# lz4/lz4-java

Measured on NVIDIA H100. Metric: lz4_fast_compress_plus_decompress_64KiB_blocks, higher is better.
Workload: dtype u8

## Files before the change

### lz4-java_b200/csrc/lz4_compress_wide.cuh

```cuda
#pragma once
#include "common.cuh"
#include "lz4_emit.cuh"
#include <type_traits>

namespace b200 {

#ifdef B200_HOST_SIM
__device__ __forceinline__ void wide_bar_arrive(int id) { simt::bar_arrive(id, 64); }
__device__ __forceinline__ void wide_bar_wait(int id) { simt::bar_sync(id, 64); }
__device__ __forceinline__ uint32_t ldg_u32(const uint32_t* p) { return *p; }
__device__ __forceinline__ void ldg_pair(const uint32_t* base, uint32_t idx, uint32_t& lo, uint32_t& hi) { lo = base[idx]; hi = base[idx + 1]; }
__device__ __forceinline__ uint2 ldg_u64(const uint2* p) { return *p; }
#else
#define B200_WBAR_CASE(OP, N) case N: asm volatile(OP " " #N ", 64;" ::: "memory"); break;
__device__ __forceinline__ void wide_bar_arrive(int id)
{
    switch (id) { B200_WBAR_CASE("bar.arrive", 1) B200_WBAR_CASE("bar.arrive", 2) B200_WBAR_CASE("bar.arrive", 3)
                  B200_WBAR_CASE("bar.arrive", 4) B200_WBAR_CASE("bar.arrive", 5) default: asm volatile("bar.arrive 6, 64;" ::: "memory"); }
}
__device__ __forceinline__ void wide_bar_wait(int id)
{
    switch (id) { B200_WBAR_CASE("bar.sync", 1) B200_WBAR_CASE("bar.sync", 2) B200_WBAR_CASE("bar.sync", 3)
                  B200_WBAR_CASE("bar.sync", 4) B200_WBAR_CASE("bar.sync", 5) default: asm volatile("bar.sync 6, 64;" ::: "memory"); }
}
__device__ __forceinline__ uint32_t ldg_u32(const uint32_t* p) { return __ldg(p); }
__device__ __forceinline__ uint2 ldg_u64(const uint2* p) { return __ldg(p); }
__device__ __forceinline__ void ldg_pair(const uint32_t* base, uint32_t idx, uint32_t& lo, uint32_t& hi)
{
    uint64_t a;
    asm("mad.wide.u32 %0, %1, 4, %2;" : "=l"(a) : "r"(idx), "l"(base));
    asm("ld.global.nc.u32 %0, [%1];" : "=r"(lo) : "l"(a));
    asm("ld.global.nc.u32 %0, [%1+4];" : "=r"(hi) : "l"(a));
}
#endif

template <int S, int NB, int NW>
struct WideLayout {
    static constexpr int CH = 128 * S;
    static constexpr int MW = CH / 32;
    static constexpr int BUF_BYTES = CH * 3 + MW * 4;
    static constexpr int REC_BYTES = 32 * 8 + 16;
    static constexpr size_t smem(int hash_log) { return (size_t(2) << hash_log) + size_t(NB) * BUF_BYTES + REC_BYTES; }
};

template <int HASH_LOG, int S, int NB, int NW, int MINB>
__global__ void __launch_bounds__(32 * NW, MINB)
lz4_compress_wide_kernel(const uint8_t* __restrict__ src_base, const uint64_t* __restrict__ src_off,
                         const int32_t* __restrict__ src_len,
                         uint8_t* __restrict__ dst_base, const uint64_t* __restrict__ dst_off,
                         const int32_t* __restrict__ dst_cap, int32_t* __restrict__ result, uint32_t nblocks)
{
    using LY = WideLayout<S, NB, NW>;
    constexpr int CH = LY::CH, MW = LY::MW;
    constexpr int TABLE_BYTES = 2 << HASH_LOG;
    constexpr int BAR_FULL = 1, BAR_FREE = 1 + NB, BAR_REC_FULL = 1 + 2 * NB, BAR_REC_FREE = 2 + 2 * NB;
    constexpr int REC_LAST = 0x100;
    static_assert(NW == 2 || NW == 3, "two or three warps");
    static_assert(2 * NB + (NW == 3 ? 2 : 0) <= 6, "named barrier ids 1..6");
    B200_DYN_SMEM(smem_raw, 128);
    uint16_t* table = reinterpret_cast<uint16_t*>(smem_raw);
    uint8_t* bufs = smem_raw + TABLE_BYTES;
    auto dist_of = [&](int buf) { return reinterpret_cast<uint16_t*>(bufs + buf * LY::BUF_BYTES); };
    auto flen_of = [&](int buf) { return bufs + buf * LY::BUF_BYTES + CH * 2; };
    auto hmask_of = [&](int buf) { return reinterpret_cast<uint32_t*>(bufs + buf * LY::BUF_BYTES + CH * 3); };
    uint2* s_rec = reinterpret_cast<uint2*>(bufs + NB * LY::BUF_BYTES);
    int* s_hdr = reinterpret_cast<int*>(bufs + NB * LY::BUF_BYTES + 256);

    const uint32_t b = blockIdx.x;
    if (b >= nblocks) return;
    const int lane = lane_id();
    const int role = threadIdx.x >> 5;
    const uint8_t* __restrict__ src = src_base + src_off[b];
    uint8_t* __restrict__ dst = dst_base + dst_off[b];
    const int n = src_len[b];
    const int cap = dst_cap[b];

    if (n < 0 || n >= 65536 + 11 || cap < 0) { if (threadIdx.x == 0) result[b] = 0; return; }
    if (n == 0) { if (threadIdx.x == 0) { if (cap >= 1) dst[0] = 0; result[b] = cap >= 1 ? 1 : 0; } return; }

    const uint32_t ph = uint32_t(reinterpret_cast<uintptr_t>(src)) & 3u;
    const uint32_t* __restrict__ wsrc = reinterpret_cast<const uint32_t*>(reinterpret_cast<uintptr_t>(src) - ph);
    const uint32_t ph8 = uint32_t(reinterpret_cast<uintptr_t>(src)) & 7u;
    const uint2* __restrict__ qsrc = reinterpret_cast<const uint2*>(reinterpret_cast<uintptr_t>(src) - ph8);
    const int mflimit = n - 12, matchlimit = n - 5;
    const int nchunks = mflimit >= 0 ? (mflimit + int(ph)) / CH + 1 : 0;
    auto ld4 = [&](int pos) -> uint32_t {
        const uint32_t a = uint32_t(pos) + ph;
        uint32_t lo, hi;
        ldg_pair(wsrc, a >> 2, lo, hi);
        return __funnelshift_r(lo, hi, a << 3);
    };

    if (role == 0) {
        for (int i = lane; i < TABLE_BYTES / 16; i += 32) reinterpret_cast<uint4*>(table)[i] = make_uint4(0, 0, 0, 0);
        __syncwarp();
        auto lookup = [&](int c, auto edge_tag) {
            constexpr bool EDGE = decltype(edge_tag)::value;
            const int buf = c % NB;
            const int cp0 = CH * c - int(ph);
            uint32_t w0[S], w1[S], w2[S]; int cand[S][4];
            #pragma unroll
            for (int s = 0; s < S; s++) {
                const int p0 = cp0 + 128 * s + 4 * lane;
                const uint32_t* wp = wsrc + (uint32_t(CH / 4) * uint32_t(c) + 32u * uint32_t(s) + uint32_t(lane));
                w0[s] = w1[s] = w2[s] = 0;
                if (!EDGE || (p0 + 3 >= 0 && p0 <= mflimit)) { w0[s] = ldg_u32(wp); w1[s] = ldg_u32(wp + 1); w2[s] = ldg_u32(wp + 2); }
            }
            #pragma unroll
            for (int s = 0; s < S; s++) {
                const int p0 = cp0 + 128 * s + 4 * lane;
                uint32_t h[4];
                #pragma unroll
                for (int j = 0; j < 4; j++) {
                    const uint32_t sq = j ? __funnelshift_r(w0[s], w1[s], 8 * j) : w0[s];
                    h[j] = (sq * 2654435761u) >> (32 - HASH_LOG);
                    cand[s][j] = table[h[j]];
                }
                __syncwarp();
                #pragma unroll
                for (int j = 0; j < 4; j++) {
                    const int p = p0 + j;
                    if (!EDGE || (p >= 0 && p <= mflimit)) table[h[j]] = uint16_t(p);
                }
                __syncwarp();
            }
            if (c >= NB) wide_bar_wait(BAR_FREE + buf);
            uint16_t* ds = dist_of(buf);
            uint8_t* fls = flen_of(buf);
            uint32_t* hm = hmask_of(buf);
            uint32_t fl[S][4], gh[S];
            #pragma unroll
            for (int s = 0; s < S; s++) {
                const int p0 = cp0 + 128 * s + 4 * lane;
                uint32_t dd[4], nib = 0;
                #pragma unroll
                for (int j = 0; j < 4; j++) {
                    const int p = p0 + j;
                    const uint32_t sq = j ? __funnelshift_r(w0[s], w1[s], 8 * j) : w0[s];
                    const uint32_t sn = j ? __funnelshift_r(w1[s], w2[s], 8 * j) : w1[s];
                    const bool plaus = !EDGE || (p >= 0 && p <= mflimit && cand[s][j] < p);
                    const uint32_t a = uint32_t(plaus ? cand[s][j] : 0) + ph8;
                    const uint2* w = qsrc + (a >> 3);
                    const uint2 q0 = ldg_u64(w), q1 = ldg_u64(w + 1);
                    const bool up = (a & 4u) != 0;
                    const uint32_t c0 = up ? q0.y : q0.x, c1 = up ? q1.x : q0.y, c2 = up ? q1.y : q1.x;
                    const uint32_t x = __funnelshift_r(c0, c1, a << 3) ^ sq;
                    const uint32_t y = __funnelshift_r(c1, c2, a << 3) ^ sn;
                    dd[j] = EDGE ? (uint32_t(p - cand[s][j]) & 0xFFFFu) : uint32_t(p - cand[s][j]);
                    fl[s][j] = 4u + min((uint32_t(__ffs(int(y))) - 1u) >> 3, 4u);
                    if (EDGE) fl[s][j] = uint32_t(min(int(fl[s][j]), max(matchlimit - p, 4)));
                    nib |= uint32_t(plaus && x == 0) << j;
                }
                reinterpret_cast<uint2*>(ds + 128 * s)[lane] = make_uint2(dd[0] | (dd[1] << 16), dd[2] | (dd[3] << 16));
                uint32_t g = nib << (4u * (uint32_t(lane) & 7u));
                g |= __shfl_xor_sync(B200_FULL, g, 1); g |= __shfl_xor_sync(B200_FULL, g, 2); g |= __shfl_xor_sync(B200_FULL, g, 4);
                if ((lane & 7) == 0) hm[4 * s + (lane >> 3)] = g;
                gh[s] = g;
            }
            #pragma unroll
            for (int s = 0; s < S; s++) {
                uint32_t nx = __shfl_down_sync(B200_FULL, gh[s], 8);
                const uint32_t nxs = (s + 1 < S) ? __shfl_sync(B200_FULL, gh[(s + 1) % S], 0) : 0u;
                if (lane >= 24) nx = nxs;
                const uint32_t win = __funnelshift_rc(gh[s], nx, 4u * (uint32_t(lane) & 7u) + 4u);
                uint32_t out = 0;
                #pragma unroll
                for (int j = 0; j < 4; j++) {
                    const uint32_t f = fl[s][j];
                    const uint32_t mm = win >> (uint32_t(j) + f - 4u);
                    const uint32_t z = uint32_t(__ffs(int(mm))) - 1u;
                    const uint32_t code = min(f * 64u - 256u + (z < 32u ? f + z : 0u), 0xFFu);
                    out |= code << (8 * j);
                }
                reinterpret_cast<uint32_t*>(fls + 128 * s)[lane] = out;
            }
            wide_bar_arrive(BAR_FULL + buf);
        };
        for (int c = 0; c < nchunks; c++) {
            const int cp0 = CH * c - int(ph);
            if (lane < S) {
                const int pfq = cp0 + 2 * CH + lane * 128;
                if (pfq < n) B200_PREFETCH_L2(src + pfq);
            }
            if (c > 0 && cp0 + CH - 1 < mflimit) lookup(c, std::false_type{});
            else lookup(c, std::true_type{});
        }
        return;
    }

    int ip = 0;
    int op = 0; bool fail = false;
    int k = 0;
    int r_pend = 0, r_ms = 0, r_len = 4, r_dist = 1;

    auto extend = [&](int a, int dist, int maxlen) -> int {
        int total = 0;
        for (;;) {
            const int i = total + 4 * lane;
            uint32_t x = 1;
            if (i < maxlen) x = ld4(a + i) ^ ld4(a + i - dist);
            const unsigned neq = __ballot_sync(B200_FULL, x != 0);
            if (neq) {
                const int fl = __ffs(neq) - 1;
                const uint32_t xf = __shfl_sync(B200_FULL, x, fl);
                return min(total + 4 * fl + ((__ffs(xf) - 1) >> 3), maxlen);
            }
            total += 128;
        }
    };

    auto layout = [&](int cnt) {
        const bool on = lane < cnt;
        int start = r_ms, len = r_len;
        if (on && r_ms - r_dist >= 4 && r_ms > r_pend) {
            const uint32_t x = ld4(r_ms - 4) ^ ld4(r_ms - r_dist - 4);
            const int back = x ? (__clz(x) >> 3) : 4;
            const int bk = min(back, r_ms - r_pend);
            start -= bk; len += bk;
        }
        const int lit = on ? start - r_pend : 0, mcode = len - 4;
        const int lhdr = lit >= 15 ? (lit - 15) / 255 + 1 : 0;
        const int mhdr = (on && mcode >= 15) ? (mcode - 15) / 255 + 1 : 0;
        const int size = on ? 1 + lhdr + lit + 2 + mhdr : 0;
        int incl = size;
        #pragma unroll
        for (int d = 1; d < 32; d <<= 1) { const int y = __shfl_up_sync(B200_FULL, incl, d); if (lane >= d) incl += y; }
        const int total = __shfl_sync(B200_FULL, incl, 31);
        if (fail) return;
        if (uint32_t(op) + uint32_t(total) > uint32_t(cap)) { fail = true; return; }
        const int o = op + incl - size;
        if (on) {
            uint8_t* d = dst + o;
            d[0] = uint8_t((min(lit, 15) << 4) | min(mcode, 15));
            d += 1;
            if (lit >= 15) { int v = lit - 15; for (; v >= 255; v -= 255) *d++ = 255; *d++ = uint8_t(v); }
            d += lit;
            d[0] = uint8_t(r_dist); d[1] = uint8_t(r_dist >> 8);
            d += 2;
            if (mcode >= 15) { int v = mcode - 15; for (; v >= 255; v -= 255) *d++ = 255; *d++ = uint8_t(v); }
        }
        uint8_t* lo = dst + o + 1 + lhdr;
        const int sn = min(lit, 32);
        const int mx = __reduce_max_sync(B200_FULL, sn);
        for (int t = 0; t < mx; t += 4) {
            if (t < sn) {
                const uint32_t v = ld4(r_pend + t);
                lo[t] = uint8_t(v);
                if (t + 1 < sn) lo[t + 1] = uint8_t(v >> 8);
                if (t + 2 < sn) lo[t + 2] = uint8_t(v >> 16);
                if (t + 3 < sn) lo[t + 3] = uint8_t(v >> 24);
            }
        }
        for (unsigned lm = __ballot_sync(B200_FULL, lit > 32); lm; lm &= lm - 1) {
            const int j = __ffs(lm) - 1;
            const int ka = __shfl_sync(B200_FULL, r_pend, j);
            const int kl = __shfl_sync(B200_FULL, lit, j);
            const int ko = __shfl_sync(B200_FULL, o + 1 + lhdr, j);
            warp_copy(dst + ko + 32, src + ka + 32, kl - 32, lane);
        }
        op += total;
    };

    auto finish = [&](int fin) {
        int ret = 0;
        if (!fail) {
            const int lit = n - fin;
            const int lhdr = lit >= 15 ? (lit - 15) / 255 + 1 : 0;
            if (uint32_t(op) + 1u + uint32_t(lhdr) + uint32_t(lit) <= uint32_t(cap)) {
                if (lane == 0) dst[op] = uint8_t(min(lit, 15) << 4);
                op += 1;
                if (lhdr) { write_len_ext(dst + op, lit - 15, lhdr, lane); op += lhdr; }
                warp_copy(dst + op, src + fin, lit, lane);
                ret = op + lit;
            }
        }
        if (lane == 0) result[b] = ret;
    };

    int prev_end = 0;
    auto layout_batch = [&](int cnt) {
        uint2 r = make_uint2(0, 4);
        if (lane < cnt) r = s_rec[lane];
        if (NW == 3) wide_bar_arrive(BAR_REC_FREE);
        r_ms = int(r.x & 0xFFFFu); r_dist = int(r.x >> 16); r_len = int(r.y);
        const int end = r_ms + r_len;
        r_pend = __shfl_up_sync(B200_FULL, end, 1);
        if (lane == 0) r_pend = prev_end;
        if (cnt > 0) prev_end = __shfl_sync(B200_FULL, end, cnt - 1);
        layout(cnt);
    };

    if (NW == 3 && role == 2) {
        for (;;) {
            wide_bar_wait(BAR_REC_FULL);
            const int hdr = s_hdr[0], fin = s_hdr[1];
            layout_batch(hdr & 0xFF);
            if (hdr & REC_LAST) { finish(fin); break; }
        }
        return;
    }

    auto flush = [&](bool last) {
        if (NW == 2) { __syncwarp(); layout_batch(k); k = 0; __syncwarp(); return; }
        if (lane == 0) { s_hdr[0] = k | (last ? REC_LAST : 0); s_hdr[1] = ip; }
        wide_bar_arrive(BAR_REC_FULL);
        wide_bar_wait(BAR_REC_FREE);
        k = 0;
    };
    for (int c = 0; c < nchunks; c++) {
        const int buf = c % NB;
        const int cp0 = CH * c - int(ph);
        wide_bar_wait(BAR_FULL + buf);
        const uint16_t* ds = dist_of(buf);
        const uint8_t* fls = flen_of(buf);
        const uint32_t* hm = hmask_of(buf);
        auto search = [&](uint32_t r) -> uint32_t {
            if (r >= uint32_t(CH)) return CH;
            uint32_t w = r >> 5;
            uint32_t m = hm[w] & (0xFFFFFFFFu << (r & 31u));
            while (m == 0 && ++w < uint32_t(MW)) m = hm[w];
            return m ? 32u * w + uint32_t(__ffs(int(m))) - 1u : uint32_t(CH);
        };
        uint32_t q = search(uint32_t(max(ip - cp0, 0)));
        uint32_t code = 0, dist = 0;
        if (q < uint32_t(CH)) { code = fls[q]; dist = ds[q]; }
        while (q < uint32_t(CH)) {
            const uint32_t ms = uint32_t(cp0) + q;
            uint32_t fl = 4u + (code >> 6);
            const uint32_t delta = code & 63u;
            uint32_t nq = q + delta;
            if (delta - 1u >= 62u) {
                if (delta) fl = 8u + uint32_t(extend(int(ms) + 8, int(dist), matchlimit - (int(ms) + 8)));
                nq = search(q + fl);
            }
            const uint32_t ncode = fls[nq], ndist = ds[nq];
            if (lane == 0) s_rec[k] = make_uint2(ms | (dist << 16), fl);
            ip = int(ms + fl);
            q = nq; code = ncode; dist = ndist;
            if (++k == 32) flush(false);
        }
        if (c + NB < nchunks) wide_bar_arrive(BAR_FREE + buf);
    }
    flush(true);
    if (NW == 2) finish(ip);
}

}
```

### lz4-java_b200/csrc/lz4_compress.cu

```cuda
#include "common.cuh"
#include "kernels.h"
#include "lz4_emit.cuh"
#include "lz4_compress_wide.cuh"
#include <type_traits>
#include <algorithm>

#ifndef B200_WIDE_WARPS
#define B200_WIDE_WARPS 3
#endif

namespace b200 {

template <int HASH_LOG, bool U16>
__global__ void __launch_bounds__(32)
lz4_compress_long_kernel(const uint8_t* __restrict__ src_base, const uint64_t* __restrict__ src_off,
                          const int32_t* __restrict__ src_len,
                          uint8_t* __restrict__ dst_base, const uint64_t* __restrict__ dst_off,
                          const int32_t* __restrict__ dst_cap, int32_t* __restrict__ result, uint32_t nblocks)
{
    using Entry = typename std::conditional<U16, uint16_t, uint32_t>::type;
    constexpr int TABLE_BYTES = int(sizeof(Entry) << HASH_LOG);
    B200_DYN_SMEM(smem_raw, 128);
    Entry* table = reinterpret_cast<Entry*>(smem_raw);
    uint16_t* s_dist = reinterpret_cast<uint16_t*>(smem_raw + TABLE_BYTES);

    const uint32_t b = blockIdx.x;
    if (b >= nblocks) return;
    const int lane = lane_id();
    const uint8_t* __restrict__ src = src_base + src_off[b];
    uint8_t* __restrict__ dst = dst_base + dst_off[b];
    const int n = src_len[b];
    const int cap = dst_cap[b];
    int ret = 0;

    if (n < 0 || n > 0x7E000000 || cap < 0) goto done;
    if (U16 && n >= 65536 + 11) goto done;
    if (n == 0) { if (cap >= 1) { if (lane == 0) dst[0] = 0; ret = 1; } goto done; }
    {
        for (int i = lane; i < TABLE_BYTES / 16; i += 32) reinterpret_cast<uint4*>(table)[i] = make_uint4(0, 0, 0, 0);
        __syncwarp();
        const uint32_t ph = uint32_t(reinterpret_cast<uintptr_t>(src)) & 3u;
        const uint32_t* __restrict__ wsrc = reinterpret_cast<const uint32_t*>(reinterpret_cast<uintptr_t>(src) - ph);
        auto ld4 = [&](int pos) -> uint32_t {
            const uint32_t a = uint32_t(pos) + ph;
            const uint32_t* w = wsrc + (a >> 2);
            return __funnelshift_r(w[0], w[1], (a & 3u) * 8u);
        };
        const int mflimit = n - 12, matchlimit = n - 5;
        int op = 0, anchor = 0, ip = 0;
        int nrec = 0, r_o = 0, r_lit = 0, r_ml = 0, r_dist = 0;

        auto flush = [&]() {
            if (lane < nrec) {
                const int mcode = r_ml - 4;
                uint8_t* d = dst + r_o;
                d[0] = uint8_t((min(r_lit, 15) << 4) | min(mcode, 15));
                d += 1;
                if (r_lit >= 15) { int v = r_lit - 15; for (; v >= 255; v -= 255) *d++ = 255; *d++ = uint8_t(v); }
                d += r_lit;
                d[0] = uint8_t(r_dist); d[1] = uint8_t(r_dist >> 8);
                d += 2;
                if (mcode >= 15) { int v = mcode - 15; for (; v >= 255; v -= 255) *d++ = 255; *d++ = uint8_t(v); }
            }
            nrec = 0;
        };

        const int nchunks = (mflimit + int(ph)) / 128 + 1;
        for (int c = 0; c < nchunks; c++) {
            const int cp0 = 128 * c - int(ph);
            if (lane < 2) {
                const int pfq = cp0 + 512 + lane * 128;
                if (pfq < n) B200_PREFETCH_L2(src + pfq);
            }
            const int p0 = cp0 + 4 * lane;
            uint32_t w0 = 0, w1 = 0;
            if (p0 + 3 >= 0 && p0 <= mflimit) { w0 = wsrc[32 * c + lane]; w1 = wsrc[32 * c + lane + 1]; }
            uint32_t seq[4], h[4]; int cand[4]; bool plaus[4];
            seq[0] = w0; seq[1] = __funnelshift_r(w0, w1, 8); seq[2] = __funnelshift_r(w0, w1, 16); seq[3] = __funnelshift_r(w0, w1, 24);
            #pragma unroll
            for (int j = 0; j < 4; j++) { h[j] = (seq[j] * 2654435761u) >> (32 - HASH_LOG); cand[j] = table[h[j]]; }
            __syncwarp();
            #pragma unroll
            for (int j = 0; j < 4; j++) {
                const int p = p0 + j;
                const bool valid = p >= 0 && p <= mflimit;
                if (valid) table[h[j]] = Entry(p);
                plaus[j] = valid && cand[j] < p && (U16 || p - cand[j] <= 65535);
            }
            uint32_t cseq[4];
            #pragma unroll
            for (int j = 0; j < 4; j++) cseq[j] = plaus[j] ? ld4(cand[j]) : ~seq[j];
            uint32_t nib = 0; uint32_t d01, d23;
            {
                uint32_t dd[4];
                #pragma unroll
                for (int j = 0; j < 4; j++) {
                    const bool hit = cseq[j] == seq[j];
                    dd[j] = hit ? uint32_t(p0 + j - cand[j]) : 0u;
                    nib |= uint32_t(hit) << j;
                }
                d01 = dd[0] | (dd[1] << 16); d23 = dd[2] | (dd[3] << 16);
            }
            reinterpret_cast<uint2*>(s_dist)[lane] = make_uint2(d01, d23);
            uint32_t gw = nib << (4 * (lane & 7));
            gw |= __shfl_xor_sync(B200_FULL, gw, 1); gw |= __shfl_xor_sync(B200_FULL, gw, 2); gw |= __shfl_xor_sync(B200_FULL, gw, 4);
            const uint32_t hw0 = __shfl_sync(B200_FULL, gw, 0), hw1 = __shfl_sync(B200_FULL, gw, 8),
                           hw2 = __shfl_sync(B200_FULL, gw, 16), hw3 = __shfl_sync(B200_FULL, gw, 24);
            const unsigned long long hlo = (unsigned long long)hw0 | ((unsigned long long)hw1 << 32);
            const unsigned long long hhi = (unsigned long long)hw2 | ((unsigned long long)hw3 << 32);
            __syncwarp();
            for (;;) {
                int r = ip - cp0;
                if (r < 0) r = 0;
                if (r >= 128) break;
                int q;
                {
                    const unsigned long long lo = r < 64 ? (hlo >> r) : 0ull;
                    if (lo) q = r + __ffsll((long long)lo) - 1;
                    else {
                        const int r2 = max(r - 64, 0);
                        const unsigned long long hi = hhi >> r2;
                        if (hi == 0) break;
                        q = 64 + r2 + __ffsll((long long)hi) - 1;
                    }
                }
                int ms = cp0 + q;
                const int dist = s_dist[q];
                int mc = ms - dist, ml;
                {
                    const int d = lane - 8;
                    const int backroom = min(ms - anchor, mc);
                    const bool ok = d < 0 ? (-d <= backroom) : (ms + d < matchlimit);
                    const bool eq = ok && src[ms + d] == src[mc + d];
                    const unsigned e = __ballot_sync(B200_FULL, eq);
                    const int back = __clz((~e) & 0xFFu) - 24;
                    const int fwd = __ffs((~(e >> 8)) | (1u << 24)) - 1;
                    ml = fwd;
                    if (fwd == 24) ml += match_extend(InGlobal{src}, ms + 24, mc + 24, matchlimit - (ms + 24), lane);
                    ms -= back; ml += back;
                }
                const int lit = ms - anchor, mcode = ml - 4;
                const int lhdr = lit >= 15 ? (lit - 15) / 255 + 1 : 0;
                const int mhdr = mcode >= 15 ? (mcode - 15) / 255 + 1 : 0;
                const int size = 1 + lhdr + lit + 2 + mhdr;
                if (uint32_t(op) + uint32_t(size) > uint32_t(cap)) goto done;
                warp_copy(dst + op + 1 + lhdr, src + anchor, lit, lane);
                if (lane == nrec) { r_o = op; r_lit = lit; r_ml = ml; r_dist = dist; }
                nrec++;
                if (nrec == 32) flush();
                op += size;
                ip = anchor = ms + ml;
            }
        }
        flush();
        {
            const int lit = n - anchor;
            const int lhdr = lit >= 15 ? (lit - 15) / 255 + 1 : 0;
            if ((long long)op + 1 + lhdr + lit > cap) goto done;
            if (lane == 0) dst[op] = uint8_t(min(lit, 15) << 4);
            op += 1;
            if (lhdr) { write_len_ext(dst + op, lit - 15, lhdr, lane); op += lhdr; }
            warp_copy(dst + op, src + anchor, lit, lane);
            op += lit;
        }
        ret = op;
    }
done:
    if (lane == 0) result[b] = ret;
}

#ifndef B200_HOST_SIM
template <int HASH_LOG, bool U16>
static cudaError_t launch_long(const BatchArgs& a, cudaStream_t st)
{
    const size_t smem = ((U16 ? 2u : 4u) << HASH_LOG) + 128 * sizeof(uint16_t);
    auto k = lz4_compress_long_kernel<HASH_LOG, U16>;
    cudaError_t e = cudaFuncSetAttribute(k, cudaFuncAttributeMaxDynamicSharedMemorySize, (int)smem);
    if (e != cudaSuccess) return e;
    cudaFuncSetAttribute(k, cudaFuncAttributePreferredSharedMemoryCarveout, cudaSharedmemCarveoutMaxShared);
    k<<<(unsigned)a.n, 32, smem, st>>>(a.src_base, a.src_off, a.src_len, a.dst_base, a.dst_off, a.dst_cap,
                                       a.result, (uint32_t)a.n);
    return cudaGetLastError();
}
#endif


#ifndef B200_HOST_SIM
template <int HASH_LOG, int NB, int NW>
static cudaError_t launch_wide(const BatchArgs& a, cudaStream_t st)
{
    constexpr int S = 2;
    using LY = WideLayout<S, NB, NW>;
    const size_t smem = LY::smem(HASH_LOG);
    constexpr int FIT = 233472 / (int(LY::smem(HASH_LOG)) + 1024);
    constexpr int MINB = FIT < 16 ? FIT : 16;
    auto k = lz4_compress_wide_kernel<HASH_LOG, S, NB, NW, MINB>;
    cudaError_t e = cudaFuncSetAttribute(k, cudaFuncAttributeMaxDynamicSharedMemorySize, (int)smem);
    if (e != cudaSuccess) return e;
    cudaFuncSetAttribute(k, cudaFuncAttributePreferredSharedMemoryCarveout, cudaSharedmemCarveoutMaxShared);
    k<<<(unsigned)a.n, 32 * NW, smem, st>>>(a.src_base, a.src_off, a.src_len, a.dst_base, a.dst_off, a.dst_cap, a.result, (uint32_t)a.n);
    return cudaGetLastError();
}


cudaError_t launch_compress_fast(const BatchArgs& a, int max_src_len, cudaStream_t st)
{
    if (a.n == 0) return cudaSuccess;
    if (max_src_len > 0 && max_src_len <= 65536) return launch_wide<13, 2, B200_WIDE_WARPS>(a, st);
    return launch_long<12, false>(a, st);
}
#endif

}
```

Before: 62.75.

## Replace per-position match bitmap handoff with compacted match-entry lists

The lookup warp now compacts the verified match candidates of each chunk into a packed list. Each entry holds position, distance, length and a skip count. Previously it wrote dense per-position distance, code and hit-mask arrays. The parse warp walks this list and uses a ballot scan to find the next entry, replacing the bitmap word search. This cuts shared-memory traffic and the skipping logic in the serial parse loop, at the cost of ballots and prefix counts in the producer plus an extra split handoff when a chunk has too many hits. Optional clock instrumentation macros are added but compiled out by default.

Result: no change. 63.18, median of 6 (+0.7%).

```diff
diff --git a/lz4-java_b200/csrc/lz4_compress_wide.cuh b/lz4-java_b200/csrc/lz4_compress_wide.cuh
--- a/lz4-java_b200/csrc/lz4_compress_wide.cuh
+++ b/lz4-java_b200/csrc/lz4_compress_wide.cuh
@@ -34,11 +34,23 @@
 }
 #endif
 
+enum { WCLK_L_TOTAL, WCLK_L_FREE, WCLK_P_TOTAL, WCLK_P_FULL, WCLK_P_EXTEND, WCLK_P_SEARCH, WCLK_P_REC_FREE, WCLK_E_REC_FULL, WCLK_N };
+#ifdef B200_WIDE_CLOCKS
+__device__ unsigned long long* b200_wide_clocks;
+#define WCLK_DECL long long wclk_[WCLK_N] = {}
+#define WCLK(k, ...) do { const long long t0_ = clock64(); __VA_ARGS__; wclk_[k] += clock64() - t0_; } while (0)
+#define WCLK_STORE(lo, hi) do { if (lane == 0) for (int k_ = (lo); k_ < (hi); k_++) b200_wide_clocks[size_t(blockIdx.x) * WCLK_N + k_] += wclk_[k_]; } while (0)
+#else
+#define WCLK_DECL
+#define WCLK(k, ...) do { __VA_ARGS__; } while (0)
+#define WCLK_STORE(lo, hi) do { } while (0)
+#endif
+
 template <int S, int NB, int NW>
 struct WideLayout {
     static constexpr int CH = 128 * S;
-    static constexpr int MW = CH / 32;
-    static constexpr int BUF_BYTES = CH * 3 + MW * 4;
+    static constexpr int CAP = 200;
+    static constexpr int BUF_BYTES = CAP * 4 + 8;
     static constexpr int REC_BYTES = 32 * 8 + 16;
     static constexpr size_t smem(int hash_log) { return (size_t(2) << hash_log) + size_t(NB) * BUF_BYTES + REC_BYTES; }
 };
@@ -51,18 +63,17 @@
                          const int32_t* __restrict__ dst_cap, int32_t* __restrict__ result, uint32_t nblocks)
 {
     using LY = WideLayout<S, NB, NW>;
-    constexpr int CH = LY::CH, MW = LY::MW;
+    constexpr int CH = LY::CH, CAP = LY::CAP;
     constexpr int TABLE_BYTES = 2 << HASH_LOG;
     constexpr int BAR_FULL = 1, BAR_FREE = 1 + NB, BAR_REC_FULL = 1 + 2 * NB, BAR_REC_FREE = 2 + 2 * NB;
     constexpr int REC_LAST = 0x100;
     static_assert(NW == 2 || NW == 3, "two or three warps");
     static_assert(2 * NB + (NW == 3 ? 2 : 0) <= 6, "named barrier ids 1..6");
+    static_assert(CH <= 256 && 128 <= CAP, "entry positions take 8 bits; a sub-round's hits fit in one buffer");
     B200_DYN_SMEM(smem_raw, 128);
     uint16_t* table = reinterpret_cast<uint16_t*>(smem_raw);
     uint8_t* bufs = smem_raw + TABLE_BYTES;
-    auto dist_of = [&](int buf) { return reinterpret_cast<uint16_t*>(bufs + buf * LY::BUF_BYTES); };
-    auto flen_of = [&](int buf) { return bufs + buf * LY::BUF_BYTES + CH * 2; };
-    auto hmask_of = [&](int buf) { return reinterpret_cast<uint32_t*>(bufs + buf * LY::BUF_BYTES + CH * 3); };
+    auto ent_of = [&](int buf) { return reinterpret_cast<uint32_t*>(bufs + buf * LY::BUF_BYTES); };
     uint2* s_rec = reinterpret_cast<uint2*>(bufs + NB * LY::BUF_BYTES);
     int* s_hdr = reinterpret_cast<int*>(bufs + NB * LY::BUF_BYTES + 256);
 
@@ -91,12 +102,13 @@
         return __funnelshift_r(lo, hi, a << 3);
     };
 
+    WCLK_DECL;
     if (role == 0) {
         for (int i = lane; i < TABLE_BYTES / 16; i += 32) reinterpret_cast<uint4*>(table)[i] = make_uint4(0, 0, 0, 0);
         __syncwarp();
+        int handoffs = 0;
         auto lookup = [&](int c, auto edge_tag) {
             constexpr bool EDGE = decltype(edge_tag)::value;
-            const int buf = c % NB;
             const int cp0 = CH * c - int(ph);
             uint32_t w0[S], w1[S], w2[S]; int cand[S][4];
             #pragma unroll
@@ -124,15 +136,11 @@
                 }
                 __syncwarp();
             }
-            if (c >= NB) wide_bar_wait(BAR_FREE + buf);
-            uint16_t* ds = dist_of(buf);
-            uint8_t* fls = flen_of(buf);
-            uint32_t* hm = hmask_of(buf);
-            uint32_t fl[S][4], gh[S];
+            uint32_t e[S][4], gh[S];
             #pragma unroll
             for (int s = 0; s < S; s++) {
                 const int p0 = cp0 + 128 * s + 4 * lane;
-                uint32_t dd[4], nib = 0;
+                uint32_t nib = 0;
                 #pragma unroll
                 for (int j = 0; j < 4; j++) {
                     const int p = p0 + j;
@@ -146,37 +154,62 @@
                     const uint32_t c0 = up ? q0.y : q0.x, c1 = up ? q1.x : q0.y, c2 = up ? q1.y : q1.x;
                     const uint32_t x = __funnelshift_r(c0, c1, a << 3) ^ sq;
                     const uint32_t y = __funnelshift_r(c1, c2, a << 3) ^ sn;
-                    dd[j] = EDGE ? (uint32_t(p - cand[s][j]) & 0xFFFFu) : uint32_t(p - cand[s][j]);
-                    fl[s][j] = 4u + min((uint32_t(__ffs(int(y))) - 1u) >> 3, 4u);
-                    if (EDGE) fl[s][j] = uint32_t(min(int(fl[s][j]), max(matchlimit - p, 4)));
+                    const uint32_t dd = uint32_t(p - cand[s][j]) & 0xFFFFu;
+                    uint32_t fl = 4u + min((uint32_t(__ffs(int(y))) - 1u) >> 3, 4u);
+                    if (EDGE) fl = uint32_t(min(int(fl), max(matchlimit - p, 4)));
+                    e[s][j] = uint32_t(128 * s + 4 * lane + j) | (dd << 8) | (fl << 28);
                     nib |= uint32_t(plaus && x == 0) << j;
                 }
-                reinterpret_cast<uint2*>(ds + 128 * s)[lane] = make_uint2(dd[0] | (dd[1] << 16), dd[2] | (dd[3] << 16));
                 uint32_t g = nib << (4u * (uint32_t(lane) & 7u));
                 g |= __shfl_xor_sync(B200_FULL, g, 1); g |= __shfl_xor_sync(B200_FULL, g, 2); g |= __shfl_xor_sync(B200_FULL, g, 4);
-                if ((lane & 7) == 0) hm[4 * s + (lane >> 3)] = g;
                 gh[s] = g;
             }
+            uint32_t win[S]; int pre[S], sb[S + 1];
+            sb[0] = 0;
             #pragma unroll
             for (int s = 0; s < S; s++) {
                 uint32_t nx = __shfl_down_sync(B200_FULL, gh[s], 8);
                 const uint32_t nxs = (s + 1 < S) ? __shfl_sync(B200_FULL, gh[(s + 1) % S], 0) : 0u;
                 if (lane >= 24) nx = nxs;
-                const uint32_t win = __funnelshift_rc(gh[s], nx, 4u * (uint32_t(lane) & 7u) + 4u);
-                uint32_t out = 0;
-                #pragma unroll
-                for (int j = 0; j < 4; j++) {
-                    const uint32_t f = fl[s][j];
-                    const uint32_t mm = win >> (uint32_t(j) + f - 4u);
-                    const uint32_t z = uint32_t(__ffs(int(mm))) - 1u;
-                    const uint32_t code = min(f * 64u - 256u + (z < 32u ? f + z : 0u), 0xFFu);
-                    out |= code << (8 * j);
-                }
-                reinterpret_cast<uint32_t*>(fls + 128 * s)[lane] = out;
-            }
-            wide_bar_arrive(BAR_FULL + buf);
+                win[s] = __funnelshift_rc(gh[s], nx, 4u * (uint32_t(lane) & 7u));
+                int below = 0, all = 0;
+                #pragma unroll
+                for (int j = 0; j < 4; j++) {
+                    const uint32_t bj = __ballot_sync(B200_FULL, (win[s] >> j) & 1u);
+                    below += __popc(bj & ((1u << lane) - 1u));
+                    all += __popc(bj);
+                }
+                pre[s] = sb[s] + below;
+                sb[s + 1] = sb[s] + all;
+            }
+            const bool split = sb[S] > CAP;
+            uint32_t* ent = nullptr;
+            int first = 0;
+            #pragma unroll
+            for (int s = 0; s < S; s++) {
+                if (s == 0 || split) {
+                    const int buf = handoffs % NB;
+                    if (handoffs >= NB) WCLK(WCLK_L_FREE, wide_bar_wait(BAR_FREE + buf));
+                    ent = ent_of(buf);
+                    first = split ? sb[s] : 0;
+                }
+                int o = pre[s] - first;
+                #pragma unroll
+                for (int j = 0; j < 4; j++) {
+                    if ((win[s] >> j) & 1u) {
+                        const uint32_t f = e[s][j] >> 28;
+                        const uint32_t skip = 1u + uint32_t(__popc((win[s] >> (j + 1)) & ((1u << (f - 1u)) - 1u)));
+                        ent[o++] = e[s][j] | (skip << 24);
+                    }
+                }
+                if (s == S - 1 || split) {
+                    if (lane == 0) ent[CAP] = uint32_t(sb[split ? s + 1 : S] - first) | (s == S - 1 ? 0x10000u : 0u);
+                    wide_bar_arrive(BAR_FULL + handoffs % NB);
+                    handoffs++;
+                }
+            }
         };
-        for (int c = 0; c < nchunks; c++) {
+        WCLK(WCLK_L_TOTAL, for (int c = 0; c < nchunks; c++) {
             const int cp0 = CH * c - int(ph);
             if (lane < S) {
                 const int pfq = cp0 + 2 * CH + lane * 128;
@@ -184,7 +217,9 @@
             }
             if (c > 0 && cp0 + CH - 1 < mflimit) lookup(c, std::false_type{});
             else lookup(c, std::true_type{});
-        }
+        });
+        for (int h = max(handoffs - NB, 0); h < handoffs; h++) wide_bar_wait(BAR_FREE + h % NB);
+        WCLK_STORE(WCLK_L_TOTAL, WCLK_L_FREE + 1);
         return;
     }
 
@@ -292,11 +327,12 @@
 
     if (NW == 3 && role == 2) {
         for (;;) {
-            wide_bar_wait(BAR_REC_FULL);
+            WCLK(WCLK_E_REC_FULL, wide_bar_wait(BAR_REC_FULL));
             const int hdr = s_hdr[0], fin = s_hdr[1];
             layout_batch(hdr & 0xFF);
             if (hdr & REC_LAST) { finish(fin); break; }
         }
+        WCLK_STORE(WCLK_E_REC_FULL, WCLK_E_REC_FULL + 1);
         return;
     }
 
@@ -304,45 +340,52 @@
         if (NW == 2) { __syncwarp(); layout_batch(k); k = 0; __syncwarp(); return; }
         if (lane == 0) { s_hdr[0] = k | (last ? REC_LAST : 0); s_hdr[1] = ip; }
         wide_bar_arrive(BAR_REC_FULL);
-        wide_bar_wait(BAR_REC_FREE);
+        WCLK(WCLK_P_REC_FREE, wide_bar_wait(BAR_REC_FREE));
         k = 0;
     };
-    for (int c = 0; c < nchunks; c++) {
-        const int buf = c % NB;
+    int handoffs = 0;
+    WCLK(WCLK_P_TOTAL, for (int c = 0; c < nchunks; c++) {
         const int cp0 = CH * c - int(ph);
-        wide_bar_wait(BAR_FULL + buf);
-        const uint16_t* ds = dist_of(buf);
-        const uint8_t* fls = flen_of(buf);
-        const uint32_t* hm = hmask_of(buf);
-        auto search = [&](uint32_t r) -> uint32_t {
-            if (r >= uint32_t(CH)) return CH;
-            uint32_t w = r >> 5;
-            uint32_t m = hm[w] & (0xFFFFFFFFu << (r & 31u));
-            while (m == 0 && ++w < uint32_t(MW)) m = hm[w];
-            return m ? 32u * w + uint32_t(__ffs(int(m))) - 1u : uint32_t(CH);
-        };
-        uint32_t q = search(uint32_t(max(ip - cp0, 0)));
-        uint32_t code = 0, dist = 0;
-        if (q < uint32_t(CH)) { code = fls[q]; dist = ds[q]; }
-        while (q < uint32_t(CH)) {
-            const uint32_t ms = uint32_t(cp0) + q;
-            uint32_t fl = 4u + (code >> 6);
-            const uint32_t delta = code & 63u;
-            uint32_t nq = q + delta;
-            if (delta - 1u >= 62u) {
-                if (delta) fl = 8u + uint32_t(extend(int(ms) + 8, int(dist), matchlimit - (int(ms) + 8)));
-                nq = search(q + fl);
-            }
-            const uint32_t ncode = fls[nq], ndist = ds[nq];
-            if (lane == 0) s_rec[k] = make_uint2(ms | (dist << 16), fl);
-            ip = int(ms + fl);
-            q = nq; code = ncode; dist = ndist;
-            if (++k == 32) flush(false);
-        }
-        if (c + NB < nchunks) wide_bar_arrive(BAR_FREE + buf);
-    }
+        uint32_t hdr;
+        do {
+            const int buf = handoffs % NB;
+            WCLK(WCLK_P_FULL, wide_bar_wait(BAR_FULL + buf));
+            const uint32_t* ent = ent_of(buf);
+            hdr = ent[CAP];
+            const int cnt = int(hdr & 0xFFFFu);
+            auto search = [&](int i0, uint32_t r) -> int {
+                if (r >= uint32_t(CH)) return cnt;
+                for (int i = i0; i < cnt; i += 32) {
+                    const unsigned m = __ballot_sync(B200_FULL, i + lane < cnt && (ent[i + lane] & 0xFFu) >= r);
+                    if (m) return i + __ffs(int(m)) - 1;
+                }
+                return cnt;
+            };
+            int i;
+            WCLK(WCLK_P_SEARCH, i = search(0, uint32_t(max(ip - cp0, 0))));
+            uint32_t e = ent[i];
+            while (i < cnt) {
+                const uint32_t q = e & 0xFFu, dist = (e >> 8) & 0xFFFFu;
+                const uint32_t ms = uint32_t(cp0) + q;
+                uint32_t fl = e >> 28;
+                int ni = i + int((e >> 24) & 15u);
+                if (fl == 8u) {
+                    WCLK(WCLK_P_EXTEND, fl = 8u + uint32_t(extend(int(ms) + 8, int(dist), matchlimit - (int(ms) + 8))));
+                    WCLK(WCLK_P_SEARCH, ni = search(i + 1, q + fl));
+                }
+                const uint32_t ne = ent[ni];
+                if (lane == 0) s_rec[k] = make_uint2(ms | (dist << 16), fl);
+                ip = int(ms + fl);
+                i = ni; e = ne;
+                if (++k == 32) flush(false);
+            }
+            wide_bar_arrive(BAR_FREE + buf);
+            handoffs++;
+        } while (!(hdr & 0x10000u));
+    });
     flush(true);
     if (NW == 2) finish(ip);
-}
-
-}
+    WCLK_STORE(WCLK_P_TOTAL, WCLK_P_REC_FREE + 1);
+}
+
+}
```

## Add hash-tag filter to skip implausible candidate loads in wide compressor

Applied to the files above, without the earlier changes.

Adds a per-hash-slot tag array (8 bits by default) in shared memory holding extra hash bits of the last inserted sequence. A candidate's global-memory verification load is issued only when its tag matches, which is meant to cut wasted global loads on hash collisions. Candidate loads also change from two 64-bit loads to one or two 128-bit loads. The change also adds optional clock64 tracing under a macro. In exchange it costs more shared memory (which may lower CTAs per SM), extra tag reads and writes, and another warp sync per sub-chunk.

After: 62.50 before, 68.79 after, median of 6. 1.1x the previous value.

```diff
diff --git a/lz4-java_b200/csrc/lz4_compress.cu b/lz4-java_b200/csrc/lz4_compress.cu
--- a/lz4-java_b200/csrc/lz4_compress.cu
+++ b/lz4-java_b200/csrc/lz4_compress.cu
@@ -186,18 +186,31 @@
 
 
 #ifndef B200_HOST_SIM
-template <int HASH_LOG, int NB, int NW>
+#ifdef B200_WIDE_TRACE
+static int g_wide_ctas_per_sm = 0;
+extern "C" int b200lz4_wide_trace_read(unsigned long long* host, int rows)
+{
+    if (rows < 0 || rows > WIDE_TRACE_ROWS) return -1;
+    return cudaMemcpyFromSymbol(host, g_wide_trace, size_t(rows) * WT_N * sizeof(unsigned long long)) == cudaSuccess ? WT_N : -1;
+}
+extern "C" int b200lz4_wide_trace_ctas_per_sm() { return g_wide_ctas_per_sm; }
+#endif
+
+template <int HASH_LOG, int NB, int NW, int TAG_BITS>
 static cudaError_t launch_wide(const BatchArgs& a, cudaStream_t st)
 {
     constexpr int S = 2;
-    using LY = WideLayout<S, NB, NW>;
+    using LY = WideLayout<S, NB, NW, TAG_BITS>;
     const size_t smem = LY::smem(HASH_LOG);
     constexpr int FIT = 233472 / (int(LY::smem(HASH_LOG)) + 1024);
     constexpr int MINB = FIT < 16 ? FIT : 16;
-    auto k = lz4_compress_wide_kernel<HASH_LOG, S, NB, NW, MINB>;
+    auto k = lz4_compress_wide_kernel<HASH_LOG, S, NB, NW, MINB, TAG_BITS>;
     cudaError_t e = cudaFuncSetAttribute(k, cudaFuncAttributeMaxDynamicSharedMemorySize, (int)smem);
     if (e != cudaSuccess) return e;
     cudaFuncSetAttribute(k, cudaFuncAttributePreferredSharedMemoryCarveout, cudaSharedmemCarveoutMaxShared);
+#ifdef B200_WIDE_TRACE
+    cudaOccupancyMaxActiveBlocksPerMultiprocessor(&g_wide_ctas_per_sm, k, 32 * NW, smem);
+#endif
     k<<<(unsigned)a.n, 32 * NW, smem, st>>>(a.src_base, a.src_off, a.src_len, a.dst_base, a.dst_off, a.dst_cap, a.result, (uint32_t)a.n);
     return cudaGetLastError();
 }
@@ -206,7 +219,7 @@
 cudaError_t launch_compress_fast(const BatchArgs& a, int max_src_len, cudaStream_t st)
 {
     if (a.n == 0) return cudaSuccess;
-    if (max_src_len > 0 && max_src_len <= 65536) return launch_wide<13, 2, B200_WIDE_WARPS>(a, st);
+    if (max_src_len > 0 && max_src_len <= 65536) return launch_wide<13, 2, B200_WIDE_WARPS, B200_WIDE_TAG_BITS>(a, st);
     return launch_long<12, false>(a, st);
 }
 #endif
diff --git a/lz4-java_b200/csrc/lz4_compress_wide.cuh b/lz4-java_b200/csrc/lz4_compress_wide.cuh
--- a/lz4-java_b200/csrc/lz4_compress_wide.cuh
+++ b/lz4-java_b200/csrc/lz4_compress_wide.cuh
@@ -2,6 +2,10 @@
 #include "common.cuh"
 #include "lz4_emit.cuh"
 #include <type_traits>
+
+#ifndef B200_WIDE_TAG_BITS
+#define B200_WIDE_TAG_BITS 8
+#endif
 
 namespace b200 {
 
@@ -10,7 +14,8 @@
 __device__ __forceinline__ void wide_bar_wait(int id) { simt::bar_sync(id, 64); }
 __device__ __forceinline__ uint32_t ldg_u32(const uint32_t* p) { return *p; }
 __device__ __forceinline__ void ldg_pair(const uint32_t* base, uint32_t idx, uint32_t& lo, uint32_t& hi) { lo = base[idx]; hi = base[idx + 1]; }
-__device__ __forceinline__ uint2 ldg_u64(const uint2* p) { return *p; }
+__device__ __forceinline__ uint4 ldg_u128(const uint4* p) { return *p; }
+__device__ __forceinline__ void shared_xor(uint32_t* p, uint32_t v) { *p ^= v; }
 #else
 #define B200_WBAR_CASE(OP, N) case N: asm volatile(OP " " #N ", 64;" ::: "memory"); break;
 __device__ __forceinline__ void wide_bar_arrive(int id)
@@ -24,7 +29,8 @@
                   B200_WBAR_CASE("bar.sync", 4) B200_WBAR_CASE("bar.sync", 5) default: asm volatile("bar.sync 6, 64;" ::: "memory"); }
 }
 __device__ __forceinline__ uint32_t ldg_u32(const uint32_t* p) { return __ldg(p); }
-__device__ __forceinline__ uint2 ldg_u64(const uint2* p) { return __ldg(p); }
+__device__ __forceinline__ uint4 ldg_u128(const uint4* p) { return __ldg(p); }
+__device__ __forceinline__ void shared_xor(uint32_t* p, uint32_t v) { atomicXor(p, v); }
 __device__ __forceinline__ void ldg_pair(const uint32_t* base, uint32_t idx, uint32_t& lo, uint32_t& hi)
 {
     uint64_t a;
@@ -34,32 +40,58 @@
 }
 #endif
 
-template <int S, int NB, int NW>
+#ifdef B200_WIDE_TRACE
+enum { WT_L_TOTAL, WT_L_FREE, WT_E_TOTAL, WT_E_REC_FULL, WT_P_TOTAL, WT_P_FULL, WT_P_REC_FREE, WT_P_EXTEND, WT_P_SEARCH,
+       WT_SEQUENCES, WT_EXTENDS, WT_SEARCHES, WT_N };
+constexpr int WIDE_TRACE_EVERY = 64, WIDE_TRACE_ROWS = 16384;
+__device__ unsigned long long g_wide_trace[WIDE_TRACE_ROWS][WT_N];
+#define WT_BEGIN unsigned long long wt[WT_N] = {}; const long long wt_start = clock64()
+#define WT_TIME(slot, ...) do { const long long t_ = clock64(); __VA_ARGS__; wt[slot] += clock64() - t_; } while (0)
+#define WT_COUNT(slot) (wt[slot] += 1)
+#define WT_END(total, lo, hi) do {                                                                                   \
+        wt[total] = clock64() - wt_start;                                                                           \
+        if (lane == 0 && b % WIDE_TRACE_EVERY == 0 && b / WIDE_TRACE_EVERY < WIDE_TRACE_ROWS) {                     \
+            g_wide_trace[b / WIDE_TRACE_EVERY][total] = wt[total];                                                 \
+            for (int i_ = lo; i_ < hi; i_++) g_wide_trace[b / WIDE_TRACE_EVERY][i_] = wt[i_];                      \
+        } } while (0)
+#else
+#define WT_BEGIN
+#define WT_TIME(slot, ...) do { __VA_ARGS__; } while (0)
+#define WT_COUNT(slot)
+#define WT_END(total, lo, hi)
+#endif
+
+template <int S, int NB, int NW, int TAG_BITS>
 struct WideLayout {
     static constexpr int CH = 128 * S;
     static constexpr int MW = CH / 32;
     static constexpr int BUF_BYTES = CH * 3 + MW * 4;
     static constexpr int REC_BYTES = 32 * 8 + 16;
-    static constexpr size_t smem(int hash_log) { return (size_t(2) << hash_log) + size_t(NB) * BUF_BYTES + REC_BYTES; }
+    static constexpr size_t tag_bytes(int hash_log) { return (size_t(TAG_BITS) << hash_log) / 8; }
+    static constexpr size_t smem(int hash_log)
+    { return (size_t(2) << hash_log) + tag_bytes(hash_log) + size_t(NB) * BUF_BYTES + REC_BYTES; }
 };
 
-template <int HASH_LOG, int S, int NB, int NW, int MINB>
+template <int HASH_LOG, int S, int NB, int NW, int MINB, int TAG_BITS = B200_WIDE_TAG_BITS>
 __global__ void __launch_bounds__(32 * NW, MINB)
 lz4_compress_wide_kernel(const uint8_t* __restrict__ src_base, const uint64_t* __restrict__ src_off,
                          const int32_t* __restrict__ src_len,
                          uint8_t* __restrict__ dst_base, const uint64_t* __restrict__ dst_off,
                          const int32_t* __restrict__ dst_cap, int32_t* __restrict__ result, uint32_t nblocks)
 {
-    using LY = WideLayout<S, NB, NW>;
+    using LY = WideLayout<S, NB, NW, TAG_BITS>;
     constexpr int CH = LY::CH, MW = LY::MW;
     constexpr int TABLE_BYTES = 2 << HASH_LOG;
+    constexpr int TAG_BYTES = int(LY::tag_bytes(HASH_LOG));
     constexpr int BAR_FULL = 1, BAR_FREE = 1 + NB, BAR_REC_FULL = 1 + 2 * NB, BAR_REC_FREE = 2 + 2 * NB;
     constexpr int REC_LAST = 0x100;
     static_assert(NW == 2 || NW == 3, "two or three warps");
     static_assert(2 * NB + (NW == 3 ? 2 : 0) <= 6, "named barrier ids 1..6");
+    static_assert(TAG_BITS == 0 || TAG_BITS == 1 || TAG_BITS == 2 || TAG_BITS == 4 || TAG_BITS == 8, "tag widths 0, 1, 2, 4, 8");
     B200_DYN_SMEM(smem_raw, 128);
     uint16_t* table = reinterpret_cast<uint16_t*>(smem_raw);
-    uint8_t* bufs = smem_raw + TABLE_BYTES;
+    uint8_t* tags = smem_raw + TABLE_BYTES;
+    uint8_t* bufs = smem_raw + TABLE_BYTES + TAG_BYTES;
     auto dist_of = [&](int buf) { return reinterpret_cast<uint16_t*>(bufs + buf * LY::BUF_BYTES); };
     auto flen_of = [&](int buf) { return bufs + buf * LY::BUF_BYTES + CH * 2; };
     auto hmask_of = [&](int buf) { return reinterpret_cast<uint32_t*>(bufs + buf * LY::BUF_BYTES + CH * 3); };
@@ -77,11 +109,12 @@
 
     if (n < 0 || n >= 65536 + 11 || cap < 0) { if (threadIdx.x == 0) result[b] = 0; return; }
     if (n == 0) { if (threadIdx.x == 0) { if (cap >= 1) dst[0] = 0; result[b] = cap >= 1 ? 1 : 0; } return; }
+    WT_BEGIN;
 
     const uint32_t ph = uint32_t(reinterpret_cast<uintptr_t>(src)) & 3u;
     const uint32_t* __restrict__ wsrc = reinterpret_cast<const uint32_t*>(reinterpret_cast<uintptr_t>(src) - ph);
-    const uint32_t ph8 = uint32_t(reinterpret_cast<uintptr_t>(src)) & 7u;
-    const uint2* __restrict__ qsrc = reinterpret_cast<const uint2*>(reinterpret_cast<uintptr_t>(src) - ph8);
+    const uint32_t ph16 = uint32_t(reinterpret_cast<uintptr_t>(src)) & 15u;
+    const uint4* __restrict__ osrc = reinterpret_cast<const uint4*>(reinterpret_cast<uintptr_t>(src) - ph16);
     const int mflimit = n - 12, matchlimit = n - 5;
     const int nchunks = mflimit >= 0 ? (mflimit + int(ph)) / CH + 1 : 0;
     auto ld4 = [&](int pos) -> uint32_t {
@@ -92,13 +125,20 @@
     };
 
     if (role == 0) {
+        constexpr uint32_t TMASK = (1u << TAG_BITS) - 1u;
+        auto tag_of = [](uint32_t prod) { return (prod >> (32 - HASH_LOG - TAG_BITS)) & TMASK; };
+        uint32_t* tagw = reinterpret_cast<uint32_t*>(tags);
+        auto tag_get = [&](uint32_t h) { return (tagw[(TAG_BITS * h) >> 5] >> ((TAG_BITS * h) & 31u)) & TMASK; };
+        const uint32_t tag0 = (TAG_BITS && nchunks) ? tag_of(ld4(0) * 2654435761u) * (0xFFFFFFFFu / max(TMASK, 1u)) : 0u;
         for (int i = lane; i < TABLE_BYTES / 16; i += 32) reinterpret_cast<uint4*>(table)[i] = make_uint4(0, 0, 0, 0);
+        for (int i = lane; i < TAG_BYTES / 16; i += 32) reinterpret_cast<uint4*>(tags)[i] = make_uint4(tag0, tag0, tag0, tag0);
         __syncwarp();
         auto lookup = [&](int c, auto edge_tag) {
             constexpr bool EDGE = decltype(edge_tag)::value;
             const int buf = c % NB;
             const int cp0 = CH * c - int(ph);
             uint32_t w0[S], w1[S], w2[S]; int cand[S][4];
+            uint32_t tok = TAG_BITS ? 0u : 0xFFFFFFFFu;
             #pragma unroll
             for (int s = 0; s < S; s++) {
                 const int p0 = cp0 + 128 * s + 4 * lane;
@@ -110,11 +150,18 @@
             for (int s = 0; s < S; s++) {
                 const int p0 = cp0 + 128 * s + 4 * lane;
                 uint32_t h[4];
+                [[maybe_unused]] uint32_t t[4], ct[4];
                 #pragma unroll
                 for (int j = 0; j < 4; j++) {
                     const uint32_t sq = j ? __funnelshift_r(w0[s], w1[s], 8 * j) : w0[s];
-                    h[j] = (sq * 2654435761u) >> (32 - HASH_LOG);
+                    const uint32_t prod = sq * 2654435761u;
+                    h[j] = prod >> (32 - HASH_LOG);
                     cand[s][j] = table[h[j]];
+                    if constexpr (TAG_BITS > 0) {
+                        t[j] = tag_of(prod);
+                        ct[j] = tag_get(h[j]);
+                        tok |= uint32_t(ct[j] == t[j]) << (4 * s + j);
+                    }
                 }
                 __syncwarp();
                 #pragma unroll
@@ -123,8 +170,19 @@
                     if (!EDGE || (p >= 0 && p <= mflimit)) table[h[j]] = uint16_t(p);
                 }
                 __syncwarp();
-            }
-            if (c >= NB) wide_bar_wait(BAR_FREE + buf);
+                if constexpr (TAG_BITS > 0) {
+                    #pragma unroll
+                    for (int j = 0; j < 4; j++) {
+                        const int p = p0 + j;
+                        if ((!EDGE || (p >= 0 && p <= mflimit)) && table[h[j]] == uint16_t(p)) {
+                            if constexpr (TAG_BITS == 8) tags[h[j]] = uint8_t(t[j]);
+                            else if (ct[j] != t[j]) shared_xor(&tagw[(TAG_BITS * h[j]) >> 5], (ct[j] ^ t[j]) << ((TAG_BITS * h[j]) & 31u));
+                        }
+                    }
+                    __syncwarp();
+                }
+            }
+            if (c >= NB) WT_TIME(WT_L_FREE, wide_bar_wait(BAR_FREE + buf));
             uint16_t* ds = dist_of(buf);
             uint8_t* fls = flen_of(buf);
             uint32_t* hm = hmask_of(buf);
@@ -138,10 +196,15 @@
                     const int p = p0 + j;
                     const uint32_t sq = j ? __funnelshift_r(w0[s], w1[s], 8 * j) : w0[s];
                     const uint32_t sn = j ? __funnelshift_r(w1[s], w2[s], 8 * j) : w1[s];
-                    const bool plaus = !EDGE || (p >= 0 && p <= mflimit && cand[s][j] < p);
-                    const uint32_t a = uint32_t(plaus ? cand[s][j] : 0) + ph8;
-                    const uint2* w = qsrc + (a >> 3);
-                    const uint2 q0 = ldg_u64(w), q1 = ldg_u64(w + 1);
+                    const bool plaus = (!EDGE || (p >= 0 && p <= mflimit && cand[s][j] < p)) && ((tok >> (4 * s + j)) & 1u);
+                    const uint32_t a = uint32_t(cand[s][j]) + ph16;
+                    const uint4* w = osrc + (a >> 4);
+                    uint4 v = make_uint4(0, 0, 0, 0), v2 = make_uint4(0, 0, 0, 0);
+                    if (plaus) v = ldg_u128(w);
+                    if (plaus && (a & 15u) > 8u) v2 = ldg_u128(w + 1);
+                    const bool h8 = (a & 8u) != 0;
+                    const uint2 q0 = h8 ? make_uint2(v.z, v.w) : make_uint2(v.x, v.y);
+                    const uint2 q1 = h8 ? make_uint2(v2.x, v2.y) : make_uint2(v.z, v.w);
                     const bool up = (a & 4u) != 0;
                     const uint32_t c0 = up ? q0.y : q0.x, c1 = up ? q1.x : q0.y, c2 = up ? q1.y : q1.x;
                     const uint32_t x = __funnelshift_r(c0, c1, a << 3) ^ sq;
@@ -185,6 +248,7 @@
             if (c > 0 && cp0 + CH - 1 < mflimit) lookup(c, std::false_type{});
             else lookup(c, std::true_type{});
         }
+        WT_END(WT_L_TOTAL, WT_L_FREE, WT_L_FREE + 1);
         return;
     }
 
@@ -292,11 +356,12 @@
 
     if (NW == 3 && role == 2) {
         for (;;) {
-            wide_bar_wait(BAR_REC_FULL);
+            WT_TIME(WT_E_REC_FULL, wide_bar_wait(BAR_REC_FULL));
             const int hdr = s_hdr[0], fin = s_hdr[1];
             layout_batch(hdr & 0xFF);
             if (hdr & REC_LAST) { finish(fin); break; }
         }
+        WT_END(WT_E_TOTAL, WT_E_REC_FULL, WT_E_REC_FULL + 1);
         return;
     }
 
@@ -304,13 +369,13 @@
         if (NW == 2) { __syncwarp(); layout_batch(k); k = 0; __syncwarp(); return; }
         if (lane == 0) { s_hdr[0] = k | (last ? REC_LAST : 0); s_hdr[1] = ip; }
         wide_bar_arrive(BAR_REC_FULL);
-        wide_bar_wait(BAR_REC_FREE);
+        WT_TIME(WT_P_REC_FREE, wide_bar_wait(BAR_REC_FREE));
         k = 0;
     };
     for (int c = 0; c < nchunks; c++) {
         const int buf = c % NB;
         const int cp0 = CH * c - int(ph);
-        wide_bar_wait(BAR_FULL + buf);
+        WT_TIME(WT_P_FULL, wide_bar_wait(BAR_FULL + buf));
         const uint16_t* ds = dist_of(buf);
         const uint8_t* fls = flen_of(buf);
         const uint32_t* hm = hmask_of(buf);
@@ -321,7 +386,8 @@
             while (m == 0 && ++w < uint32_t(MW)) m = hm[w];
             return m ? 32u * w + uint32_t(__ffs(int(m))) - 1u : uint32_t(CH);
         };
-        uint32_t q = search(uint32_t(max(ip - cp0, 0)));
+        uint32_t q;
+        WT_TIME(WT_P_SEARCH, q = search(uint32_t(max(ip - cp0, 0)))); WT_COUNT(WT_SEARCHES);
         uint32_t code = 0, dist = 0;
         if (q < uint32_t(CH)) { code = fls[q]; dist = ds[q]; }
         while (q < uint32_t(CH)) {
@@ -330,19 +396,21 @@
             const uint32_t delta = code & 63u;
             uint32_t nq = q + delta;
             if (delta - 1u >= 62u) {
-                if (delta) fl = 8u + uint32_t(extend(int(ms) + 8, int(dist), matchlimit - (int(ms) + 8)));
-                nq = search(q + fl);
+                if (delta) { WT_TIME(WT_P_EXTEND, fl = 8u + uint32_t(extend(int(ms) + 8, int(dist), matchlimit - (int(ms) + 8)))); WT_COUNT(WT_EXTENDS); }
+                WT_TIME(WT_P_SEARCH, nq = search(q + fl)); WT_COUNT(WT_SEARCHES);
             }
             const uint32_t ncode = fls[nq], ndist = ds[nq];
             if (lane == 0) s_rec[k] = make_uint2(ms | (dist << 16), fl);
             ip = int(ms + fl);
             q = nq; code = ncode; dist = ndist;
+            WT_COUNT(WT_SEQUENCES);
             if (++k == 32) flush(false);
         }
         if (c + NB < nchunks) wide_bar_arrive(BAR_FREE + buf);
     }
     flush(true);
     if (NW == 2) finish(ip);
+    WT_END(WT_P_TOTAL, WT_P_FULL, WT_N);
 }
 
 }
```
